# Thraix/VoxelRayTracer

Hardware: AMD Instinct MI355X
Metric: Mrays/sec + achieved HBM GB/s, 1920x1080 @ 128^3 voxels, 4 bounces (higher is better)
Workload: dtype f32

## Files before the change

voxelraytracer_amd/csrc/vrt_cert.h:

```cpp
#ifndef VRT_CERT_H
#define VRT_CERT_H

#include "vrt_walk.h"

namespace vrt {


enum : int { CERT_MISS = 0, CERT_HIT = 1, CERT_UNSURE = 2 };
constexpr int kCertRun = 3;
constexpr float kCertMargin = 1.0f / 64.0f;
constexpr int kCertMaxIter = 1024;
constexpr float kCertMaxOrigin = 4e-3f;

struct CertResult {
  int res;
  uint32_t byte;
  int axis;
  int cx, cy, cz;
  float u;
  float eu;
  float us;
  CERT_DIAG_ONLY(int iters;)
};

// ... 12 lines not shown
  uint32_t t = load_u16_at(c.vox, outside ? 0u : idx, obase);
  t = outside ? kTexOutside : t;
  asm volatile("" : "+v"(t));
  return t;
}
__device__ __forceinline__ bool cross_outside(uint32_t tex) { return tex >= kTexOutside; }
__device__ __forceinline__ uint32_t start_texel(const Ctx& c, int i, int j, int k, uint32_t obase) {
  const bool outside = max(max(uint32_t(i), uint32_t(j)), uint32_t(k)) >= uint32_t(c.n);
  const uint32_t idx = mad24(mad24(uint32_t(k), c.p, uint32_t(j)), c.p, uint32_t(i));
  const uint32_t t = load_u16_at(c.vox, outside ? 0u : idx, obase);
  return outside ? 0u : t;
}
__device__ __forceinline__ uint32_t alt_byte(const Ctx& c, int i, int j, int k, uint32_t obase) {
  const uint32_t n = uint32_t(c.n);
  if (uint32_t(i) > n || uint32_t(j) > n || uint32_t(k) > n) return 0u;
  return cell_texel(c, i, j, k, obase) & kVoxMask;
}
template <bool SHADOW>
__device__ __forceinline__ bool cert_event(uint32_t b, uint32_t medium) {
  return SHADOW ? (b & ~2u) != 0u : b != medium;
}

struct CertStartK {
  f3 Ps, fl;
  int mx, my, mz;
};
typedef const __attribute__((address_space(4))) KArgs LateKArgs;
__device__ __forceinline__ LateKArgs* late_kargs() {
  LateKArgs* ka = (LateKArgs*)__builtin_amdgcn_kernarg_segment_ptr();
  asm volatile("" : "+s"(ka));
  return ka;
}

template <bool SHADOW, bool LEAN = false, bool ED = true>
__device__ __forceinline__ CertResult cert_walk(const Ctx& c, const f3 P, const f3 D, const f3 rcp, const float U,
                                int cx, int cy, int cz, const float e0, const f3 ed,
                                const float len0b, const uint32_t medium, const uint32_t tex0 = ~0u,
                                const CertStartK* __restrict__ st0 = nullptr,
                                LateKArgs* sk = nullptr) {
  CertResult r;
  r.res = CERT_UNSURE;
  r.byte = 0u;
  r.axis = 0;
  r.cx = r.cy = r.cz = 0;
  r.u = 0.0f;
  r.eu = 0.0f;
  r.us = 0.0f;
  const bool ksun = LEAN && sk != nullptr;
  const int sx = ksun ? sk->sun_step[0] : (D.x > 0.0f ? 1 : -1), sy = ksun ? sk->sun_step[1] : (D.y > 0.0f ? 1 : -1),
            sz = ksun ? sk->sun_step[2] : (D.z > 0.0f ? 1 : -1);
  const int ux = ksun ? (sk->sun_step[0] > 0 ? 1 : 0) : (D.x > 0.0f ? 1 : 0), uy = ksun ? (sk->sun_step[1] > 0 ? 1 : 0) : (D.y > 0.0f ? 1 : 0),
            uz = ksun ? (sk->sun_step[2] > 0 ? 1 : 0) : (D.z > 0.0f ? 1 : 0);
  const f3 ar = mk(__builtin_fabsf(rcp.x), __builtin_fabsf(rcp.y), __builtin_fabsf(rcp.z));
  const float l1 = ksun ? sk->sun_l1 : __builtin_fabsf(D.x) + __builtin_fabsf(D.y) + __builtin_fabsf(D.z);
  const uint32_t obase =
      ksun ? sk->sun_obase : ((D.x < 0.0f ? 1u : 0u) | (D.y < 0.0f ? 2u : 0u) | (D.z < 0.0f ? 4u : 0u)) * c.ostride;
  constexpr float k24 = 2.0f * 0x1p-24f;
  const float q2 = ksun ? sk->sun_q2 : 0.5f * k24 * l1;
  const float lin = 6.0f + l1 * (len0b + 1.0f),
              con = (18.0f * 1.0000020f) * __builtin_amdgcn_rcpf(l1) + 3.0f * (len0b + 1.0f);
  const float a1 = k24 * (lin + 2.0f), b1 = ksun ? sk->sun_b1 : k24 * l1, b0 = k24 * (3.0f * c.fn + 11.0f);
  const float c0 = k24 * (con + 2.0f * len0b) + 4e-5f + e0;
  const float g2 = ksun ? sk->sun_g2 : 2.0f * q2, g1 = 2.0f * k24 * lin, g0 = 2.0f * k24 * con + 1e-4f + e0;
  const bool kst = LEAN && st0 != nullptr;
  const f3 Ps = kst    ? st0->Ps
                : ksun ? mk(__uint_as_float(__float_as_uint(P.x) ^ sk->sun_neg[0]), __uint_as_float(__float_as_uint(P.y) ^ sk->sun_neg[1]),
                            __uint_as_float(__float_as_uint(P.z) ^ sk->sun_neg[2]))
                       : mk(ux ? P.x : -P.x, uy ? P.y : -P.y, uz ? P.z : -P.z);
  const f3 Da = mk(__builtin_fabsf(D.x), __builtin_fabsf(D.y), __builtin_fabsf(D.z));
  const int mx = kst ? st0->mx : ux - 1, my = kst ? st0->my : uy - 1, mz = kst ? st0->mz : uz - 1;
  f3 sig = kst ? mk(((st0->fl.x + 1.0f) - Ps.x) * ar.x, ((st0->fl.y + 1.0f) - Ps.y) * ar.y,
                    ((st0->fl.z + 1.0f) - Ps.z) * ar.z)
               : mk((float(cx + ux) - P.x) * rcp.x, (float(cy + uy) - P.y) * rcp.y, (float(cz + uz) - P.z) * rcp.z);
  uint32_t tex = (tex0 != ~0u ? tex0
                              : (LEAN ? start_texel(c, cx + sx, cy + sy, cz + sz, obase)
                                      : path_texel(c, cx + sx, cy + sy, cz + sz, obase))) +
                 (1u << kDistShift);
  CTRACE(c, 100 + int(SHADOW), cx, cy, cz, P.x, P.y, P.z, U);
  CTRACE(c, 101, D.x, D.y, D.z, e0, ed.x, ed.y, ed.z);
  CERT_DIAG_ONLY(r.iters = 0;)
  if (LEAN && PHASE_STOP(SHADOW ? 4 : 2)) {
    r.u = ((sig.x + sig.y) + (sig.z + q2)) + ((a1 + b1) + (b0 + c0)) + ((g2 + g1) + (g0 + Ps.x)) +
          ((Ps.y + Ps.z) + (Da.x + Da.y)) + ((Da.z + ar.x) + (ar.y + ar.z)) + U;
    r.cx = int(tex + obase) + mx + my + mz;
    return r;
  }
  int st = CERT_UNSURE;
  for (int guard = 0; guard < kCertMaxIter; ++guard) {
    CERT_DIAG_ONLY(r.iters = guard + 1;)
    const float s1 = __builtin_fminf(sig.x, __builtin_fminf(sig.y, sig.z));
    const float uu = gmax(s1, 0.0f);
    const float A = __builtin_fmaf(__builtin_fmaf(q2, uu, a1), uu, c0);
    const float B = __builtin_fmaf(b1, uu, b0);
    auto gam_of = [&](float arb, float edb) {
      const float g = __builtin_fmaf(B, arb, A);
      return ED ? g + edb : g;
    };
    const uint32_t G = tex >> kDistShift;
    bool jumped = false;
    if (SHADOW || medium == 0u) {
      const float fg1 = float(G) - (1.0f + kCertMargin);
      const float fb = fg1 - B;
      const float jx = __builtin_fmaf(fb, ar.x, sig.x), jy = __builtin_fmaf(fb, ar.y, sig.y),
                  jz = __builtin_fmaf(fb, ar.z, sig.z);
      const float jm = ED ? __builtin_fminf(jx - ed.x, __builtin_fminf(jy - ed.y, jz - ed.z))
                          : __builtin_fminf(jx, __builtin_fminf(jy, jz));
      const float uj = __builtin_fminf(jm - A, U + 2.0f);
      CTRACE(c, 102, G, s1, uj, gam_of(ar.x, ed.x), gam_of(ar.y, ed.y), gam_of(ar.z, ed.z), 0);
      if (uj > s1) {
        const float fx = __builtin_floorf(__builtin_fmaf(uj, Da.x, Ps.x)),
                    fy = __builtin_floorf(__builtin_fmaf(uj, Da.y, Ps.y)),
                    fz = __builtin_floorf(__builtin_fmaf(uj, Da.z, Ps.z));
        cx = int(fx) ^ mx;
        cy = int(fy) ^ my;
        cz = int(fz) ^ mz;
        if constexpr (LEAN)
          sig = mk(((fx + 1.0f) - Ps.x) * ar.x, ((fy + 1.0f) - Ps.y) * ar.y, ((fz + 1.0f) - Ps.z) * ar.z);
        else
          sig = mk((float(cx + ux) - P.x) * rcp.x, (float(cy + uy) - P.y) * rcp.y, (float(cz + uz) - P.z) * rcp.z);
        tex = LEAN ? cell_texel(c, cx, cy, cz, obase) : path_texel(c, cx, cy, cz, obase);
        jumped = true;
      }
    }
    st = kCertRun;
    if (!jumped) {
      const int a = sig.x == s1 ? 0 : (sig.y == s1 ? 1 : 2);
      const f3 gam = mk(gam_of(ar.x, ed.x), gam_of(ar.y, ed.y), gam_of(ar.z, ed.z));
      const f3 back = mk(sig.x - ar.x, sig.y - ar.y, sig.z - ar.z);
      const float mback = gmax(back.x, gmax(back.y, back.z));
      const float prev = gmax(mback, 0.0f);
// ... 663 lines not shown
  const float ey = h.eu * __builtin_fabsf(dy) +
                   0x1p-21f * (__builtin_fabsf(py0) + __builtin_fabsf(h.u * dy) + __builtin_fabsf(py) + 1.0f);
  uint32_t i, j;
  if (!texel_pair(c, px, ex, mat_tex_x(m), false, i) || !texel_pair(c, py, ey, mat_tex_y(m), true, j)) return false;
  const uint32_t t = c.atlas[j * (c.atlas_mask + 1u) + i];
  col = make_float4(float(t & 0xFFu) / 255.0f, float((t >> 8) & 0xFFu) / 255.0f,
                    float((t >> 16) & 0xFFu) / 255.0f, float(t >> 24) / 255.0f);
  return true;
}

__device__ __forceinline__ void late_ctx(Ctx& c) {
  LateKArgs* ka = late_kargs();
  c.sky_sy = ka->sky_sy;
  c.sun_n = mk(ka->sun_n[0], ka->sun_n[1], ka->sun_n[2]);
  c.sun_rcp = mk(ka->sun_rcp[0], ka->sun_rcp[1], ka->sun_rcp[2]);
  c.atlas = ka->atlas;
  c.atlas_mask = uint32_t(ka->atlas_size) - 1u;
  c.atlas_fs = float(ka->atlas_size);
  c.atlas_fts = float(ka->atlas_tex_size);
}
template <bool TEX = false, bool TREE = false, int NL = kWgThreads, bool LEAN = false>
__device__ __forceinline__ bool cert_pixel(const Ctx& c0, const Ray& ray0, f3& color_out, int max_refl = 0,
                                           int max_transp = 0, float* __restrict__ ltb = nullptr,
                                           float* us_out = nullptr) {
  const f3 P = ray0.pos, D = ray0.dir;
  int cx, cy, cz;
  CertStartK st;
  if constexpr (LEAN) {
    const bool ux = D.x > 0.0f, uy = D.y > 0.0f, uz = D.z > 0.0f;
    st.Ps = mk(ux ? P.x : -P.x, uy ? P.y : -P.y, uz ? P.z : -P.z);
    st.fl = mk(__builtin_floorf(st.Ps.x), __builtin_floorf(st.Ps.y), __builtin_floorf(st.Ps.z));
    st.mx = ux ? 0 : -1;
    st.my = uy ? 0 : -1;
    st.mz = uz ? 0 : -1;
    cx = int(st.fl.x) ^ st.mx;
    cy = int(st.fl.y) ^ st.my;
    cz = int(st.fl.z) ^ st.mz;
    bool ok = int(fast_path_ok(D)) & int(max(max(uint32_t(cx), uint32_t(cy)), uint32_t(cz)) < uint32_t(c0.n)) &
              int(__builtin_floorf(st.Ps.x + 1.0f) == st.fl.x + 1.0f) &
              int(__builtin_floorf(st.Ps.y + 1.0f) == st.fl.y + 1.0f) &
              int(__builtin_floorf(st.Ps.z + 1.0f) == st.fl.z + 1.0f);
    const bool on_plane = (int(!ux) & int(st.fl.x == st.Ps.x)) | (int(!uy) & int(st.fl.y == st.Ps.y)) |
                          (int(!uz) & int(st.fl.z == st.Ps.z));
    if (ok & on_plane) ok = start_layers_clear<false>(c0, P, D, cx, cy, cz, 0u);
    if (!ok) { CERT_DIAG(0); return false; }
  } else {
    if (!fast_path_ok(D)) { CERT_DIAG(0); return false; }
    if (!exact_start_cell(c0, P, D, cx, cy, cz) || !start_layers_clear<false>(c0, P, D, cx, cy, cz, 0u)) {
      CERT_DIAG(0);
      return false;
    }
  }
  const f3 rcp = mk(__builtin_amdgcn_rcpf(D.x), __builtin_amdgcn_rcpf(D.y), __builtin_amdgcn_rcpf(D.z));
  CertResult h = cert_walk<false, LEAN, false>(c0, P, D, rcp, c0.max_len - ray0.len, cx, cy, cz, 0.0f,
                                               mk(0.0f, 0.0f, 0.0f), 0.0f, 0u, ~0u, LEAN ? &st : nullptr);
  if (us_out) *us_out = h.us;
  CERT_DIAG_ONLY(cert_diag_iters(10, h.iters);)
  if (LEAN && (PHASE_STOP(2) || PHASE_STOP(3))) {
    color_out = mk(h.u, h.eu, float(h.cx + h.cy + h.cz + h.axis + int(h.byte) + h.res));
    return true;
  }
  if (h.res == CERT_UNSURE) { CERT_DIAG(1); return false; }
  Ctx c = c0;
  if constexpr (LEAN) late_ctx(c);
  f3 color = mk(0.0f, 0.0f, 0.0f);
  if (h.res == CERT_MISS) {
    CERT_DIAG(2);
// ... 25 lines not shown
```

voxelraytracer_amd/csrc/vrt_context.cpp:

```cpp
#include <hip/hip_runtime.h>
#include <rccl/rccl.h>

#include <algorithm>
#include <cmath>
#include <cstdint>
#include <cstring>
#include <string>
#include <vector>

#include "vrt.h"
#include "vrt_internal.h"

namespace {

constexpr int kParts = 2;
constexpr int kLanes = 4;
constexpr int kOrderSlots = 16;
constexpr uint32_t kOrderMaxTiles = 1u << 17;
constexpr size_t kOrderSlotWords = vrt::kOrdHdr + 5u * size_t(kOrderMaxTiles) + 2u * vrt::kOrdClasses;
uint32_t defer_seg_tiles(uint32_t tiles, uint32_t tiles_x) {
  return (tiles_x + vrt::kOrdClasses - 1u) / vrt::kOrdClasses * (tiles / tiles_x);
}
size_t defer_words(uint32_t tiles, uint32_t tiles_x) {
  return vrt::kDeferHdr + size_t(vrt::kOrdClasses) * defer_seg_tiles(tiles, tiles_x) * vrt::kWgThreads;
}
constexpr int kRing = 8;
constexpr size_t kVstatWords = 8;
static_assert(kRing % kLanes == 0, "a ring slot is always written from the same lane");

// ... 50 lines not shown
  uint64_t order_tick = 0;
  uint32_t order_assigned = 0;
};

}

void vrt::sun_consts(KArgs& a) {
  const float* s = a.sun_n;
  const float lo = 0x1p-64f, hi = 1.0e4f;
  bool ok = true;
  for (int b = 0; b < 3; ++b) ok = ok && std::fabs(s[b]) >= lo && std::fabs(s[b]) <= hi;
  a.sun_ok = ok ? 1u : 0u;
  for (int b = 0; b < 3; ++b) {
    a.sun_neg[b] = s[b] > 0.0f ? 0u : 0x80000000u;
    a.sun_step[b] = s[b] > 0.0f ? 1 : -1;
  }
  a.sun_obase = ((s[0] < 0.0f ? 1u : 0u) | (s[1] < 0.0f ? 2u : 0u) | (s[2] < 0.0f ? 4u : 0u)) * a.ostride;
  constexpr float k24 = 2.0f * 0x1p-24f;
  const float l1 = std::fabs(s[0]) + std::fabs(s[1]) + std::fabs(s[2]);
  a.sun_l1 = l1;
  a.sun_q2 = 0.5f * k24 * l1;
  a.sun_b1 = k24 * l1;
  a.sun_g2 = 2.0f * a.sun_q2;
}

struct vrt_ctx {
  std::vector<Shard> sh;
  bool distinct = true;
  bool coll1 = false;
  std::vector<ncclComm_t> comms;
  int32_t layout_req = 0;
  int32_t cert_req = 0;
  int32_t tree_req = 1;
  int tile_order = 1;
  int32_t exact_pass = 1;
  std::vector<hipEvent_t> lt_ev;
  size_t lt_used = 0;
  std::vector<uint8_t> atlas_host;
  int32_t hist_w = 0, hist_h = 0;
  uint64_t fk = 0;
  bool raw_is_cur[kRing] = {};
  bool reset_pending = false;
  uint32_t* d_gather = nullptr;
  size_t hist_pixels_gather = 0;
  uint32_t* d_frames[kRing] = {};
  hipEvent_t ev_consumed[kRing] = {};
// ... 251 lines not shown
  a.refr_noise = p->refraction_noise;
  a.max_len = p->max_ray_length;
  a.n = s.n;
  a.fn = float(s.n);
  a.width = cam->width;
  a.height = cam->height;
  a.rcp_w = 1.0f / float(cam->width);
  a.rcp_h = 1.0f / float(cam->height);
  a.row0 = row0;
  a.rows = rows;
  a.row_step = row_step;
  a.row_blk_sh = 0;
  a.pitch = cam->width;
  a.ostride = octant_stride(s);
  vrt::sun_consts(a);
  a.max_refl = p->max_reflections;
  a.max_transp = p->max_transparencies;
  a.textured = p->color_only ? 0 : 1;
  a.atlas_size = p->color_only ? 1 : p->atlas_size;
  a.atlas_tex_size = p->atlas_texture_size;
  a.atlas = s.d_atlas;
  a.alpha = 1.0f;
  a.vdiv_ok = 0;
  a.prev = nullptr;
  a.cur = nullptr;
  a.raw = nullptr;
  const bool trees = ctx->tree_req == 2 || (ctx->tree_req == 1 && !s.cert_auto);
  a.cert = s.octants != 8 || ctx->cert_req < 0 ? 0 : (ctx->cert_req > 0 || s.cert_auto || trees ? 2 : 1);
  a.tree = a.cert == 2 && p->color_only && trees ? 1 : 0;
  a.tiles_x = uint32_t((a.width + vrt::kTileW - 1) / vrt::kTileW);
  a.tiles = a.tiles_x * uint32_t((a.rows + vrt::kTileH - 1) / vrt::kTileH);
  a.order = nullptr;
  a.ord_r = a.ord_w = a.ctr_r = a.ctr_w = a.ctr_z = a.ord_q = 0;
  a.defer = nullptr;
  a.defer_e = a.defer_seg = 0;
  a.exact_fat = 0;
  a.exact_grid = 0;
  a.batches_out = nullptr;
  a.nframes = 1;
  a.frame_tiles = a.tiles;
  std::memset(a.fb, 0, sizeof(a.fb));
  return a;
}

OrderSlot* acquire_slot(Shard& s, const vrt::KArgs& a, hipStream_t st) {
  if (a.tiles == 0 || a.tiles > kOrderMaxTiles) return nullptr;
// ... 112 lines not shown
  return slot;
}

bool vertex_div_ranges_ok(const float* m) {
  const double hi = 0x1p59, lo = 0x1p-59;
  double sum[4];
  for (int i = 0; i < 4; ++i) {
    sum[i] = std::fabs(double(m[i])) + std::fabs(double(m[4 + i])) + std::fabs(double(m[8 + i])) +
             std::fabs(double(m[12 + i]));
    if (!(sum[i] * (1.0 + 0x1p-20) <= hi)) return false;
  }
  const double side = std::fabs(double(m[3])) + std::fabs(double(m[7])) + sum[3] * 0x1p-20;
  return std::fabs(double(m[15]) - double(m[11])) - side >= lo &&
         std::fabs(double(m[15]) + double(m[11])) - side >= lo;
}

void launch(const vrt_ctx* ctx, Shard& s, vrt::KArgs a, float4* out, vrt_hit* hit, unsigned long long* cnt,
            hipStream_t st, hipEvent_t ev_begin = nullptr, hipEvent_t ev_end = nullptr, bool allow_defer = true,
            bool lone = false) {
  const bool stats = hit || cnt;
  a.vdiv_ok = vertex_div_ranges_ok(a.inv_pv) ? 1u : 0u;
  for (int f = 1; f < a.nframes; ++f)
    if (!vertex_div_ranges_ok(a.fb[f - 1].inv_pv)) a.vdiv_ok = 0u;
  OrderSlot* slot = stats ? nullptr : launch_state_begin(ctx, s, a, st, allow_defer || lone, lone);
  vrt::launch_render(a, stats, s.d_vox_pad, out, hit, cnt ? s.d_cnt_rep : nullptr, st, ev_begin, ev_end);
  slot_launched(s, slot, st);
  if (cnt) vrt::launch_reduce_counters(s.d_cnt_rep, cnt, st);
}

int volume_alloc(vrt_ctx* ctx, Shard& s, int32_t n) {
  if (n < 2 || n > 1024 || (n & (n - 1)) != 0)
    return fail(ctx, VRT_ERR_INVALID, "volume edge must be a power of two in [2, 1024]");
  VRT_HIP(ctx, hipSetDevice(s.device));
  VRT_HIP(ctx, hipDeviceSynchronize());
  const bool fits = uint64_t(n + 1) * (n + 1) * (n + 1) * 2 * 8 <= (uint64_t(1) << 32);
  const int32_t octants = fits && ctx->layout_req != 1 ? 8 : 1;
  if (s.d_vox && (s.n != n || s.octants != octants)) {
    (void)hipFree(s.d_vox);
    (void)hipFree(s.d_tmp);
    (void)hipFree(s.d_vox_pad);
    s.d_vox = s.d_tmp = nullptr;
    s.d_vox_pad = nullptr;
  }
  if (!s.d_vox) {
    const size_t bytes = size_t(n) * n * n, pbytes = size_t(n + 1) * (n + 1) * (n + 1) * 2 * size_t(octants);
    if (hipMalloc(&s.d_vox, bytes) != hipSuccess ||
// ... 439 lines not shown
  if (devs.size() > 1 && c->distinct) {
    c->comms.resize(devs.size());
    if (ncclCommInitAll(c->comms.data(), int(devs.size()), devs.data()) != ncclSuccess) {
      c->comms.clear();
      vrt_destroy(c);
      return VRT_ERR_DEVICE;
    }
  }
  *out = c;
  return VRT_OK;
}

}

extern "C" {

int vrt_debug_sun_consts(const float* sun_dir, uint32_t ostride, uint32_t* out) {
  if (!sun_dir || !out) return VRT_ERR_INVALID;
  vrt::KArgs a{};
  fill_sun(a, sun_dir);
  a.ostride = ostride;
  vrt::sun_consts(a);
  std::memcpy(out, &a.sun_ok, 12 * sizeof(uint32_t));
  return VRT_OK;
}

int vrt_create(uint32_t device_mask, vrt_ctx** out) {
  std::vector<int> devs;
  for (int d = 0; d < 32; ++d)
    if (device_mask & (1u << d)) devs.push_back(d);
  if (devs.empty()) {
    if (out) *out = nullptr;
    return VRT_ERR_INVALID;
  }
  return create(devs, out);
}

int vrt_create_devices(const int32_t* devices, int32_t count, vrt_ctx** out) {
  if (!devices || count < 1) {
    if (out) *out = nullptr;
    return VRT_ERR_INVALID;
  }
  return create(std::vector<int>(devices, devices + count), out);
}

void vrt_destroy(vrt_ctx* c) {
// ... 1199 lines not shown
```

voxelraytracer_amd/csrc/vrt_internal.h:

```cpp
#ifndef VRT_INTERNAL_H
#define VRT_INTERNAL_H

#include <hip/hip_runtime.h>

#include <cstdint>

#include "vrt.h"
#include "vrt_tuning.h"

namespace vrt {

struct KArgs {
  float inv_pv[16];
  float rcp_w, rcp_h;
  float sun[3];
  float sky_sy;
  float sun_n[3];
  float sun_rcp[3];
  float time, ray_noise, refl_noise, refr_noise, max_len;
  float fn;
  int32_t n, width, height;
  int32_t row0, rows, row_step;
  int32_t row_blk_sh;
  int32_t pitch;
// ... 8 lines not shown
  uint32_t* raw;
  int32_t cert;
  int32_t tree;
  uint32_t* order;
  uint32_t tiles_x, tiles, ord_r, ord_w, ctr_r, ctr_w, ctr_z, ord_q;
  uint32_t* defer;
  uint32_t defer_e, defer_seg;
  int32_t exact_fat;
  uint32_t exact_grid;
  uint32_t* batches_out;
  int32_t nframes;
  uint32_t frame_tiles;
  struct FrameB {
    float inv_pv[16];
    float time;
    uint32_t* cur;
    uint32_t* raw;
  } fb[7];
  uint32_t sun_ok;
  uint32_t sun_neg[3];
  int32_t sun_step[3];
  uint32_t sun_obase;
  float sun_l1, sun_q2, sun_b1, sun_g2;
};
void sun_consts(KArgs& a);
constexpr int kMaxBatch = 8;
constexpr int kWgThreads = 64 * kWgWaves;
constexpr int kTileW = kWgWaves >= 2 ? 16 : 8;
constexpr int kTileH = kWgWaves == 4 ? 16 : 8;
constexpr int kMaxStack = 17;
constexpr int kCntReplicas = 256;
constexpr uint32_t kOrdClasses = 8;
constexpr uint32_t kOrdCtrStride = 64;
constexpr uint32_t kOrdHdr = 3 * kOrdClasses * kOrdCtrStride;
__host__ __device__ inline uint32_t ord_q_for(uint32_t tiles) {
  return (tiles + kOrdClasses * kOrdDiv - 1u) / (kOrdClasses * kOrdDiv);
}
constexpr uint32_t kDeferHdr = 4 * kOrdClasses * kOrdCtrStride;
constexpr uint32_t kDeferDense = 32;


void launch_render(const KArgs& a, bool stats, const uint16_t* vox, float4* out, vrt_hit* hit,
                   unsigned long long* cnt_rep, hipStream_t s, hipEvent_t ev_begin = nullptr,
                   hipEvent_t ev_end = nullptr);
constexpr int32_t kQueryPick = 2;
void launch_ray_query(const KArgs& a, int32_t kind, const uint16_t* vox, const void* in, uint32_t count,
                      vrt_ray_hit* hits, hipStream_t s, hipEvent_t ev_begin = nullptr, hipEvent_t ev_end = nullptr);
constexpr int32_t kTraceRays = 0, kTracePixels = 1;
// ... 40 lines not shown
```

voxelraytracer_amd/csrc/vrt_math.h:

```cpp
#ifndef VRT_MATH_H
#define VRT_MATH_H

#include <hip/hip_runtime.h>

#include <cstdint>

namespace vrt {


struct f3 {
  float x, y, z;
};

__device__ __forceinline__ f3 mk(float x, float y, float z) { return f3{x, y, z}; }
__device__ __forceinline__ f3 operator+(f3 a, f3 b) { return mk(a.x + b.x, a.y + b.y, a.z + b.z); }
__device__ __forceinline__ f3 operator-(f3 a, f3 b) { return mk(a.x - b.x, a.y - b.y, a.z - b.z); }
__device__ __forceinline__ f3 operator*(f3 a, float s) { return mk(a.x * s, a.y * s, a.z * s); }
__device__ __forceinline__ f3 operator*(float s, f3 a) { return mk(s * a.x, s * a.y, s * a.z); }
__device__ __forceinline__ float dot3(f3 a, f3 b) { return a.x * b.x + a.y * b.y + a.z * b.z; }
__device__ __forceinline__ float comp(f3 a, int i) { return i == 0 ? a.x : (i == 1 ? a.y : a.z); }
__device__ __forceinline__ void set_comp(f3& a, int i, float f) {
  if (i == 0) a.x = f;
  else if (i == 1) a.y = f;
  else a.z = f;
// ... 2 lines not shown
  const uint32_t e = (__float_as_uint(d) >> 23) & 0xFFu;
  return e >= 2u && e <= 252u;
}
__device__ __forceinline__ float rcp_newton(float d) {
  const float y = __builtin_amdgcn_rcpf(d);
  return __builtin_fmaf(__builtin_fmaf(-d, y, 1.0f), y, y);
}
__device__ __forceinline__ float rcp_rn(float d) { return rcp_rn_ok(d) ? rcp_newton(d) : 1.0f / d; }
__device__ __forceinline__ bool sqrt_fix_ok(float s) {
  const uint32_t e = (__float_as_uint(s) >> 23) & 0xFFu;
  return e >= 95u && e <= 252u;
}
__device__ __forceinline__ float sqrt_fix(float s) {
  const float y = __builtin_amdgcn_sqrtf(s);
  const float ym = __uint_as_float(__float_as_uint(y) - 1u), yp = __uint_as_float(__float_as_uint(y) + 1u);
  const float rm = __builtin_fmaf(-ym, y, s), rp = __builtin_fmaf(-yp, y, s);
  const float z = rm <= 0.0f ? ym : y;
  return rp > 0.0f ? yp : z;
}
__device__ __forceinline__ float sqrt_rn(float s) { return sqrt_fix_ok(s) ? sqrt_fix(s) : __builtin_sqrtf(s); }

__device__ __forceinline__ float near_one_rsqrt(uint32_t b) {
  const uint32_t one = 0x3F800000u;
  const uint32_t r = b >= one ? (b - one < 2u ? one : one - ((b - one) & ~1u))
                              : one + (((((one - b) + 1u) >> 1) + 1u) >> 1);
  return __uint_as_float(r);
}
__device__ __forceinline__ f3 normalize3(f3 v) {
  const float s = v.x * v.x + v.y * v.y + v.z * v.z;
  const uint32_t b = __float_as_uint(s);
  const float inv = b - (0x3F800000u - 1024u) <= 2048u ? near_one_rsqrt(b) : rcp_rn(sqrt_rn(s));
  return v * inv;
}
__device__ __forceinline__ float gsign(float x) { return x > 0.0f ? 1.0f : (x < 0.0f ? -1.0f : 0.0f); }
__device__ __forceinline__ float gmin(float x, float y) { return y < x ? y : x; }
__device__ __forceinline__ float gmax(float x, float y) { return __builtin_fmaxf(x, y); }
__device__ __forceinline__ float gpow(float x, float y) { return exp2f(y * log2f(x)); }
__device__ __forceinline__ float mixf(float x, float y, float a) { return x * (1.0f - a) + y * a; }
__device__ __forceinline__ f3 reflect3(f3 i, f3 n) {
  const float s = 2.0f * dot3(n, i);
  return i - s * n;
}
__device__ __forceinline__ f3 refract3(f3 i, f3 n, float eta) {
  const float d = dot3(n, i);
  const float k = 1.0f - eta * eta * (1.0f - d * d);
  if (k < 0.0f) return mk(0.0f, 0.0f, 0.0f);
  const float s = eta * d + sqrt_rn(k);
  return eta * i - s * n;
}
__device__ __forceinline__ f3 sign3(f3 d) { return mk(gsign(d.x), gsign(d.y), gsign(d.z)); }

__device__ __forceinline__ uint32_t hash1(uint32_t x) {
  x += (x << 10u);
  x ^= (x >> 6u);
  x += (x << 3u);
  x ^= (x >> 11u);
  x += (x << 15u);
  return x;
}
__device__ __forceinline__ float random4(float x, float y, float z, float w) {
  const uint32_t h = hash1(__float_as_uint(x) ^ hash1(__float_as_uint(y)) ^
                           hash1(__float_as_uint(z)) ^ hash1(__float_as_uint(w)));
  return __uint_as_float((h & 0x007FFFFFu) | 0x3F800000u) - 1.0f;
}
__device__ __forceinline__ bool zero_noise_exact(f3 d) {
  const uint32_t nz = 0x80000000u;
  return int(__float_as_uint(d.x) != nz) & int(__float_as_uint(d.y) != nz) &
         int(__float_as_uint(d.z) != nz) & int(d.x == d.x) & int(d.y == d.y) & int(d.z == d.z);
}
__device__ __forceinline__ bool zero_noise_exact_class(f3 d) {
  constexpr int kNegZeroOrNan = 0x020 | 0x001 | 0x002;
  return !(__builtin_amdgcn_classf(d.x, kNegZeroOrNan) | __builtin_amdgcn_classf(d.y, kNegZeroOrNan) |
           __builtin_amdgcn_classf(d.z, kNegZeroOrNan));
}
template <bool LEAN = false>
__device__ __forceinline__ f3 randomize(f3 dir, f3 pos, float randomness, float seed) {
  f3 r = mk(0.0f, 0.0f, 0.0f);
  if (!(randomness == 0.0f && (LEAN ? zero_noise_exact_class(dir) : zero_noise_exact(dir)))) {
    const f3 p = mk((pos.x + dir.x) + seed, (pos.y + dir.y) + seed, (pos.z + dir.z) + seed);
    const float dx = random4(p.x, p.y, p.z, 0.0f + seed);
    const float dy = random4(p.x, p.y, p.z, 0.5f + seed);
    const float dz = random4(p.x, p.y, p.z, 1.0f + seed);
    r = mk((dx + -0.5f) * randomness, (dy + -0.5f) * randomness, (dz + -0.5f) * randomness);
  }
  return normalize3(dir + r);
}


__device__ __forceinline__ uint32_t mat_id(uint32_t b) { return b > 3 ? 3 : b; }
__device__ __forceinline__ float mat_refr(uint32_t b) { return mat_id(b) == 2 ? 1.5f : 1.0f; }
__device__ __forceinline__ bool mat_transparent(uint32_t m) { return m == 0 || m == 2; }
__device__ __forceinline__ bool mat_reflective(uint32_t m) { return m == 2; }
__device__ __forceinline__ float mat_kd(uint32_t m) { return m == 0 ? 0.0f : (m == 2 ? 1.0f : 0.4f); }
__device__ __forceinline__ float mat_ks(uint32_t m, bool tex) {
  return m == 0 ? 0.0f : (m == 2 ? 1.0f : (tex ? (m == 1 ? 0.6f : 0.4f) : 0.2f));
}
__device__ __forceinline__ float mat_exp(uint32_t m, bool tex) {
  return m == 0 ? 0.0f : (m == 2 ? (tex ? 0.3f : 1.0f) : (tex ? (m == 1 ? 60.0f : 20.0f) : 10.0f));
}
__device__ __forceinline__ uint32_t mat_tex_x(uint32_t m) { return m == 3 ? 1u : 0u; }
__device__ __forceinline__ uint32_t mat_tex_y(uint32_t m) { return m >= 2 ? 1u : 0u; }
__device__ __forceinline__ float4 mat_color(uint32_t m) {
  if (m == 1) return make_float4(0.5f, 0.5f, 0.5f, 1.0f);
  if (m == 3) return make_float4(0.05f, 0.5f, 0.1f, 1.0f);
  return make_float4(0.0f, 0.0f, 0.0f, 0.0f);
}

constexpr float kAmbient = 0.3f;
// ... 7 lines not shown
```

voxelraytracer_amd/csrc/vrt_render.hip:

```cpp
#include <hip/hip_ext.h>
#include <hip/hip_runtime.h>

#include <algorithm>
#include <cmath>
#include <cstdint>
#include <cstdio>
#include <cstring>
#include <string>
#include <vector>

#include "vrt.h"
#include "vrt_internal.h"
#include "vrt_diag.h"
#include "vrt_math.h"
#include "vrt_walk.h"
#include "vrt_cert.h"
#include "vrt_aux_kernels.h"
#include "vrt_skipfield_kernels.h"

namespace vrt {

__device__ __forceinline__ uint32_t unorm8(float f) {
  const float c = __builtin_fminf(__builtin_fmaxf(f, 0.0f), 1.0f);
  return uint32_t(__builtin_rintf(c * 255.0f));
// ... 95 lines not shown
  c.refr_noise = a.refr_noise;
  if constexpr (LATE) {
    c.sky_sy = 0.0f;
    c.sun_n = c.sun_rcp = mk(0.0f, 0.0f, 0.0f);
    c.atlas = nullptr;
    c.atlas_mask = 0u;
    c.atlas_fs = c.atlas_fts = 0.0f;
  } else {
    c.sky_sy = a.sky_sy;
    c.sun_n = mk(a.sun_n[0], a.sun_n[1], a.sun_n[2]);
    c.sun_rcp = mk(a.sun_rcp[0], a.sun_rcp[1], a.sun_rcp[2]);
    c.atlas = a.atlas;
    c.atlas_mask = uint32_t(a.atlas_size) - 1u;
    c.atlas_fs = float(a.atlas_size);
    c.atlas_fts = float(a.atlas_tex_size);
  }
  CTRACE_ONLY(c.tr = false;)
}

__device__ __forceinline__ bool markstein_safe(float x) {
  const float m = __builtin_fabsf(x);
  return m >= 0x1p-60f && m <= 0x1p60f;
}
template <bool LEAN = false>
__device__ __forceinline__ f3 div3_rn(float x, float y, float z, float d, bool ranges_ok = false) {
  bool safe;
  if constexpr (LEAN) {
    bool rest = true;
    if (!ranges_ok)
      rest = int(__builtin_fabsf(x) <= 0x1p60f) & int(__builtin_fabsf(y) <= 0x1p60f) &
             int(__builtin_fabsf(z) <= 0x1p60f) & int(markstein_safe(d));
    safe = rest & (__builtin_fminf(__builtin_fminf(__builtin_fabsf(x), __builtin_fabsf(y)), __builtin_fabsf(z)) >=
                   0x1p-60f);
  } else {
    safe = markstein_safe(x) && markstein_safe(y) && markstein_safe(z) && markstein_safe(d);
  }
  if (safe) {
    const float r = rcp_newton(d);
    return mk(div_rn(x, d, r), div_rn(y, d, r), div_rn(z, d, r));
  }
  return mk(x / d, y / d, z / d);
}

template <bool LEAN = false>
__device__ __forceinline__ Ray primary_ray(const KArgs& a, const float* __restrict__ inv_pv, const Ctx& c, int px,
                                           int py) {
  const float ndx = div_rn(2.0f * (float(px) + 0.5f), float(a.width), a.rcp_w) - 1.0f;
  const float ndy = div_rn(2.0f * (float(py) + 0.5f), float(a.height), a.rcp_h) - 1.0f;
  float n4[4], f4[4];
#pragma unroll
  for (int i = 0; i < 4; ++i) {
    const float base = inv_pv[0 * 4 + i] * ndx + inv_pv[1 * 4 + i] * ndy;
    n4[i] = (base + inv_pv[2 * 4 + i] * -1.0f) + inv_pv[3 * 4 + i] * 1.0f;
    f4[i] = (base + inv_pv[2 * 4 + i] * 1.0f) + inv_pv[3 * 4 + i] * 1.0f;
  }
  const bool ranges_ok = LEAN && a.vdiv_ok != 0u;
  const f3 vnear = div3_rn<LEAN>(n4[0], n4[1], n4[2], n4[3], ranges_ok);
  const f3 vdir = div3_rn<LEAN>(f4[0], f4[1], f4[2], f4[3], ranges_ok) - vnear;
  Ray ray;
  ray.pos = mk(vnear.x + c.fn * 0.5f, vnear.y + c.fn * 0.5f, vnear.z + c.fn * 0.5f);
  ray.dir = randomize<LEAN>(normalize3(vdir), vnear, a.ray_noise, c.time);
  ray.len = 0.0f;
  ray.energy = 1.0f;
  ray.voxel = 0;
  ray.rdepth = 0;
  ray.tdepth = 0;
  return ray;
}

constexpr int kStackPrio = 3;

struct StackRay {
  f3 pos, dir;
  float len, energy;
  uint32_t depths;
};
__device__ __forceinline__ StackRay pack_stack_ray(const Ray& r) {
  return StackRay{r.pos, r.dir, r.len, r.energy, uint32_t(r.rdepth) | (uint32_t(r.tdepth) << 16)};
}
constexpr int kStackWords = 9;
template <int NL>
__device__ __forceinline__ void lds_stack_put(float* __restrict__ b, const StackRay& e) {
  b[0 * NL] = e.pos.x;
  b[1 * NL] = e.pos.y;
// ... 146 lines not shown
    constexpr int kPool = std::max(kAxFloats + kStkFloats, 4);
    __shared__ float4 lds_pool[kPool / 4];
    c.ax = &lds_pool[threadIdx.x * kAxLane];
    const Ray ray = primary_ray<DEFER>(a, FB ? frame_view(a, fr).pv : a.inv_pv, c, px, frame_row(a, li));
    k.c[VRT_CNT_PIXELS] = 1;
    k.c[VRT_CNT_PRIMARY_RAYS] = 1;
    uint32_t steps = 0, flags = 0;
    int32_t hit_vidx = -1;
    float hit_len = 0.0f;
    f3 color;
    if constexpr (!DEFER) color = mk(0.0f, 0.0f, 0.0f);
    float* tstk = nullptr;
    if constexpr (TREE) {
      static_assert(CERT == 2 && !TEX && !STATS, "certified trees: stats-free colour-only certified instances");
      tstk = reinterpret_cast<float*>(lds_pool) + kAxFloats + threadIdx.x;
    }
    float us = -1.0f;
    bool need_exact;
    if (DEFER && (PHASE_STOP(0) || PHASE_STOP(1))) {
      color = PHASE_STOP(1) ? mk(ray.pos.x + ray.dir.x, ray.pos.y + ray.dir.y, ray.pos.z + ray.dir.z)
                            : mk(0.0f, 0.0f, 0.0f);
      need_exact = false;
    } else {
      need_exact = CERT < 2 || !cert_pixel<TEX, TREE, kWgThreads, DEFER>(c, ray, color, a.max_refl, a.max_transp, tstk, &us);
    }
    STAMP_WAVE_CERT(need_exact);
    if constexpr (DEFER) {
      deferred = need_exact;
    } else if (need_exact) {
      color = mk(0.0f, 0.0f, 0.0f);
      heavy = true;
      float* lstk = reinterpret_cast<float*>(lds_pool) + kAxFloats;
      (void)exact_pixel<STATS, TEX, CERT >= 1, CERT == 2>(a, c, ray, color, k, steps, flags, hit_vidx,
                                                         hit_len, &lstk[threadIdx.x], STATS ? -1.0f : us);
    }
    const uint32_t l2 = lane_id();
    const size_t o = size_t(pixel_row(ty, wave, l2)) * size_t(a.pitch) + size_t(pixel_x(tx, wave, l2));
    if (STATS && hits) {
      vrt_hit hr;
      hr.voxel_index = hit_vidx;
      hr.ray_length = hit_len;
      hr.steps = steps;
      hr.flags = flags;
      hits[o] = hr;
    }
    if constexpr (DEFER) {
      if (!deferred) {
// ... 416 lines not shown
```

Baseline: 100,800.

## Precompute camera-invariant ray setup constants on host and pass via kernel args

After: 106,200 (median of 6 runs). +5.3%, better.

```diff
diff --git a/voxelraytracer_amd/csrc/vrt_cert.h b/voxelraytracer_amd/csrc/vrt_cert.h
--- a/voxelraytracer_amd/csrc/vrt_cert.h
+++ b/voxelraytracer_amd/csrc/vrt_cert.h
@@ -58,8 +58,9 @@
 }
 
 struct CertStartK {
-  f3 Ps, fl;
+  f3 Ps, fl1;
   int mx, my, mz;
+  float b0, U2;
 };
 typedef const __attribute__((address_space(4))) KArgs LateKArgs;
 __device__ __forceinline__ LateKArgs* late_kargs() {
@@ -83,6 +84,7 @@
   r.eu = 0.0f;
   r.us = 0.0f;
   const bool ksun = LEAN && sk != nullptr;
+  const bool kst = LEAN && st0 != nullptr;
   const int sx = ksun ? sk->sun_step[0] : (D.x > 0.0f ? 1 : -1), sy = ksun ? sk->sun_step[1] : (D.y > 0.0f ? 1 : -1),
             sz = ksun ? sk->sun_step[2] : (D.z > 0.0f ? 1 : -1);
   const int ux = ksun ? (sk->sun_step[0] > 0 ? 1 : 0) : (D.x > 0.0f ? 1 : 0), uy = ksun ? (sk->sun_step[1] > 0 ? 1 : 0) : (D.y > 0.0f ? 1 : 0),
@@ -95,18 +97,17 @@
   const float q2 = ksun ? sk->sun_q2 : 0.5f * k24 * l1;
   const float lin = 6.0f + l1 * (len0b + 1.0f),
               con = (18.0f * 1.0000020f) * __builtin_amdgcn_rcpf(l1) + 3.0f * (len0b + 1.0f);
-  const float a1 = k24 * (lin + 2.0f), b1 = ksun ? sk->sun_b1 : k24 * l1, b0 = k24 * (3.0f * c.fn + 11.0f);
+  const float a1 = k24 * (lin + 2.0f), b1 = ksun ? sk->sun_b1 : k24 * l1,
+              b0 = kst ? st0->b0 : (ksun ? sk->walk_b0 : k24 * (3.0f * c.fn + 11.0f));
   const float c0 = k24 * (con + 2.0f * len0b) + 4e-5f + e0;
   const float g2 = ksun ? sk->sun_g2 : 2.0f * q2, g1 = 2.0f * k24 * lin, g0 = 2.0f * k24 * con + 1e-4f + e0;
-  const bool kst = LEAN && st0 != nullptr;
   const f3 Ps = kst    ? st0->Ps
                 : ksun ? mk(__uint_as_float(__float_as_uint(P.x) ^ sk->sun_neg[0]), __uint_as_float(__float_as_uint(P.y) ^ sk->sun_neg[1]),
                             __uint_as_float(__float_as_uint(P.z) ^ sk->sun_neg[2]))
                        : mk(ux ? P.x : -P.x, uy ? P.y : -P.y, uz ? P.z : -P.z);
   const f3 Da = mk(__builtin_fabsf(D.x), __builtin_fabsf(D.y), __builtin_fabsf(D.z));
   const int mx = kst ? st0->mx : ux - 1, my = kst ? st0->my : uy - 1, mz = kst ? st0->mz : uz - 1;
-  f3 sig = kst ? mk(((st0->fl.x + 1.0f) - Ps.x) * ar.x, ((st0->fl.y + 1.0f) - Ps.y) * ar.y,
-                    ((st0->fl.z + 1.0f) - Ps.z) * ar.z)
+  f3 sig = kst ? mk((st0->fl1.x - Ps.x) * ar.x, (st0->fl1.y - Ps.y) * ar.y, (st0->fl1.z - Ps.z) * ar.z)
                : mk((float(cx + ux) - P.x) * rcp.x, (float(cy + uy) - P.y) * rcp.y, (float(cz + uz) - P.z) * rcp.z);
   uint32_t tex = (tex0 != ~0u ? tex0
                               : (LEAN ? start_texel(c, cx + sx, cy + sy, cz + sz, obase)
@@ -141,7 +142,7 @@
                   jz = __builtin_fmaf(fb, ar.z, sig.z);
       const float jm = ED ? __builtin_fminf(jx - ed.x, __builtin_fminf(jy - ed.y, jz - ed.z))
                           : __builtin_fminf(jx, __builtin_fminf(jy, jz));
-      const float uj = __builtin_fminf(jm - A, U + 2.0f);
+      const float uj = __builtin_fminf(jm - A, kst ? st0->U2 : U + 2.0f);
       CTRACE(c, 102, G, s1, uj, gam_of(ar.x, ed.x), gam_of(ar.y, ed.y), gam_of(ar.z, ed.z), 0);
       if (uj > s1) {
         const float fx = __builtin_floorf(__builtin_fmaf(uj, Da.x, Ps.x)),
@@ -851,27 +852,39 @@
 template <bool TEX = false, bool TREE = false, int NL = kWgThreads, bool LEAN = false>
 __device__ __forceinline__ bool cert_pixel(const Ctx& c0, const Ray& ray0, f3& color_out, int max_refl = 0,
                                            int max_transp = 0, float* __restrict__ ltb = nullptr,
-                                           float* us_out = nullptr) {
+                                           float* us_out = nullptr, const KArgs* ak = nullptr) {
   const f3 P = ray0.pos, D = ray0.dir;
   int cx, cy, cz;
   CertStartK st;
   if constexpr (LEAN) {
     const bool ux = D.x > 0.0f, uy = D.y > 0.0f, uz = D.z > 0.0f;
     st.Ps = mk(ux ? P.x : -P.x, uy ? P.y : -P.y, uz ? P.z : -P.z);
-    st.fl = mk(__builtin_floorf(st.Ps.x), __builtin_floorf(st.Ps.y), __builtin_floorf(st.Ps.z));
     st.mx = ux ? 0 : -1;
     st.my = uy ? 0 : -1;
     st.mz = uz ? 0 : -1;
-    cx = int(st.fl.x) ^ st.mx;
-    cy = int(st.fl.y) ^ st.my;
-    cz = int(st.fl.z) ^ st.mz;
-    bool ok = int(fast_path_ok(D)) & int(max(max(uint32_t(cx), uint32_t(cy)), uint32_t(cz)) < uint32_t(c0.n)) &
-              int(__builtin_floorf(st.Ps.x + 1.0f) == st.fl.x + 1.0f) &
-              int(__builtin_floorf(st.Ps.y + 1.0f) == st.fl.y + 1.0f) &
-              int(__builtin_floorf(st.Ps.z + 1.0f) == st.fl.z + 1.0f);
-    const bool on_plane = (int(!ux) & int(st.fl.x == st.Ps.x)) | (int(!uy) & int(st.fl.y == st.Ps.y)) |
-                          (int(!uz) & int(st.fl.z == st.Ps.z));
-    if (ok & on_plane) ok = start_layers_clear<false>(c0, P, D, cx, cy, cz, 0u);
+    st.b0 = ak->walk_b0;
+    st.U2 = ak->max_len2;
+    bool ok;
+    if ((ak->setup & kSetupCell) != 0u) {
+      st.fl1 = mk(ux ? ak->start_fl1[0] : ak->start_fl1[3], uy ? ak->start_fl1[1] : ak->start_fl1[4],
+                  uz ? ak->start_fl1[2] : ak->start_fl1[5]);
+      cx = ak->start_cell[0];
+      cy = ak->start_cell[1];
+      cz = ak->start_cell[2];
+      ok = fast_path_ok(D);
+    } else {
+      const f3 fl = mk(__builtin_floorf(st.Ps.x), __builtin_floorf(st.Ps.y), __builtin_floorf(st.Ps.z));
+      st.fl1 = mk(fl.x + 1.0f, fl.y + 1.0f, fl.z + 1.0f);
+      cx = int(fl.x) ^ st.mx;
+      cy = int(fl.y) ^ st.my;
+      cz = int(fl.z) ^ st.mz;
+      ok = int(fast_path_ok(D)) & int(max(max(uint32_t(cx), uint32_t(cy)), uint32_t(cz)) < uint32_t(c0.n)) &
+           int(__builtin_floorf(st.Ps.x + 1.0f) == st.fl1.x) & int(__builtin_floorf(st.Ps.y + 1.0f) == st.fl1.y) &
+           int(__builtin_floorf(st.Ps.z + 1.0f) == st.fl1.z);
+      const bool on_plane = (int(!ux) & int(fl.x == st.Ps.x)) | (int(!uy) & int(fl.y == st.Ps.y)) |
+                            (int(!uz) & int(fl.z == st.Ps.z));
+      if (ok & on_plane) ok = start_layers_clear<false>(c0, P, D, cx, cy, cz, 0u);
+    }
     if (!ok) { CERT_DIAG(0); return false; }
   } else {
     if (!fast_path_ok(D)) { CERT_DIAG(0); return false; }
diff --git a/voxelraytracer_amd/csrc/vrt_context.cpp b/voxelraytracer_amd/csrc/vrt_context.cpp
--- a/voxelraytracer_amd/csrc/vrt_context.cpp
+++ b/voxelraytracer_amd/csrc/vrt_context.cpp
@@ -5,6 +5,7 @@
 #include <cmath>
 #include <cstdint>
 #include <cstring>
+#include <limits>
 #include <string>
 #include <vector>
 
@@ -101,6 +102,82 @@
   a.sun_q2 = 0.5f * k24 * l1;
   a.sun_b1 = k24 * l1;
   a.sun_g2 = 2.0f * a.sun_q2;
+}
+
+void vrt::setup_consts(KArgs& a) {
+  constexpr float k24 = 2.0f * 0x1p-24f;
+  a.fw = float(a.width);
+  a.fh = float(a.height);
+  a.half_n = a.fn * 0.5f;
+  a.walk_b0 = k24 * (3.0f * a.fn + 11.0f);
+  a.max_len2 = a.max_len + 2.0f;
+}
+
+void vrt::cert_launch_consts(KArgs& a) {
+  a.setup = 0u;
+  a.wn = a.wf = a.rcp_wn = a.rcp_wf = 0.0f;
+  for (int i = 0; i < 6; ++i) a.start_fl1[i] = 0.0f;
+  for (int b = 0; b < 3; ++b) a.start_cell[b] = 0;
+  if (a.vdiv_ok == 0u) return;
+  for (int f = 1; f < a.nframes; ++f)
+    if (std::memcmp(a.fb[f - 1].inv_pv, a.inv_pv, sizeof(a.inv_pv)) != 0) return;
+  const float* m = a.inv_pv;
+  for (int i = 0; i < 16; ++i)
+    if (!std::isfinite(m[i])) return;
+
+  const double am11 = std::fabs(double(m[11]));
+  if (!(am11 >= double(std::numeric_limits<float>::min()))) return;
+  const double ulp = std::ldexp(1.0, std::ilogb(am11) - 23);
+  if (!((std::fabs(double(m[3])) + std::fabs(double(m[7]))) * (1.0 + 0x1p-20) < ulp * 0.25)) return;
+  const float wn = -m[11] + m[15], wf = m[11] + m[15];
+  const auto markstein = [](float x) { return std::fabs(x) >= 0x1p-60f && std::fabs(x) <= 0x1p60f; };
+  if (!markstein(wn) || !markstein(wf)) return;
+  a.wn = wn;
+  a.wf = wf;
+  a.rcp_wn = 1.0f / wn;
+  a.rcp_wf = 1.0f / wf;
+  a.setup |= kSetupW;
+
+  const double iwn = 1.0 / std::fabs(double(wn)), iwf = 1.0 / std::fabs(double(wf));
+  double S[3], en[3], ev1 = 0.0, up = 0.0;
+  double ca[3], cb[3], cc[3];
+  for (int b = 0; b < 3; ++b) {
+    S[b] = std::fabs(double(m[b])) + std::fabs(double(m[4 + b])) + std::fabs(double(m[8 + b])) +
+           std::fabs(double(m[12 + b]));
+    en[b] = 0x1p-19 * S[b] * iwn;
+    const double ef = 0x1p-19 * S[b] * iwf;
+    ev1 += 2.0 * (en[b] + ef);
+    up += S[b] * (iwn + iwf);
+    const double d = 1.0 / double(wf) - 1.0 / double(wn);
+    ca[b] = double(m[b]) * d;
+    cb[b] = double(m[4 + b]) * d;
+    cc[b] = (double(m[8 + b]) + double(m[12 + b])) / double(wf) - (double(m[12 + b]) - double(m[8 + b])) / double(wn);
+  }
+
+  const double cl = std::sqrt(cc[0] * cc[0] + cc[1] * cc[1] + cc[2] * cc[2]);
+  if (cl > 0.0 && std::isfinite(cl)) {
+    const double pa = std::fabs(ca[0] * cc[0] + ca[1] * cc[1] + ca[2] * cc[2]) / cl;
+    const double pb = std::fabs(cb[0] * cc[0] + cb[1] * cc[1] + cb[2] * cc[2]) / cl;
+    if (cl - pa - pb - ev1 >= 4.0 && up + ev1 <= 0x1p49) a.setup |= kSetupLen;
+  }
+
+  const double half = double(a.fn) * 0.5;
+  int32_t cell[3];
+  for (int b = 0; b < 3; ++b) {
+    const double centre = (double(m[12 + b]) - double(m[8 + b])) / double(wn) + half;
+    const double spread = (std::fabs(double(m[b])) + std::fabs(double(m[4 + b]))) * iwn;
+    const double e = en[b] + 0x1p-23 * (std::fabs(centre) + half + spread) + 0x1p-9;
+    const double lo = centre - spread - e, hi = centre + spread + e;
+    const double c = std::floor(lo);
+    if (!(lo > c && hi < c + 1.0 && c >= 0.0 && c < double(a.n))) return;
+    cell[b] = int32_t(c);
+  }
+  for (int b = 0; b < 3; ++b) {
+    a.start_cell[b] = cell[b];
+    a.start_fl1[b] = float(cell[b] + 1);
+    a.start_fl1[3 + b] = float(-cell[b]);
+  }
+  a.setup |= kSetupCell;
 }
 
 struct vrt_ctx {
@@ -398,6 +475,8 @@
   a.atlas = s.d_atlas;
   a.alpha = 1.0f;
   a.vdiv_ok = 0;
+  vrt::setup_consts(a);
+  vrt::cert_launch_consts(a);
   a.prev = nullptr;
   a.cur = nullptr;
   a.raw = nullptr;
@@ -556,6 +635,13 @@
   a.vdiv_ok = vertex_div_ranges_ok(a.inv_pv) ? 1u : 0u;
   for (int f = 1; f < a.nframes; ++f)
     if (!vertex_div_ranges_ok(a.fb[f - 1].inv_pv)) a.vdiv_ok = 0u;
+  vrt::cert_launch_consts(a);
+#ifdef VRT_SETUP_MASK
+#ifndef VRT_DIAGNOSTIC_BUILD
+#error "VRT_SETUP_MASK is a diagnostic build: use make variant"
+#endif
+  a.setup &= uint32_t(VRT_SETUP_MASK);
+#endif
   OrderSlot* slot = stats ? nullptr : launch_state_begin(ctx, s, a, st, allow_defer || lone, lone);
   vrt::launch_render(a, stats, s.d_vox_pad, out, hit, cnt ? s.d_cnt_rep : nullptr, st, ev_begin, ev_end);
   slot_launched(s, slot, st);
@@ -1041,6 +1127,34 @@
   a.ostride = ostride;
   vrt::sun_consts(a);
   std::memcpy(out, &a.sun_ok, 12 * sizeof(uint32_t));
+  return VRT_OK;
+}
+
+int vrt_debug_cert_launch_consts(const float* inv_pv, const float* inv_pv2, int32_t n, int32_t width, int32_t height,
+                                 float max_len, uint32_t* out) {
+  if (!inv_pv || !out) return VRT_ERR_INVALID;
+  vrt::KArgs a{};
+  std::memcpy(a.inv_pv, inv_pv, sizeof(a.inv_pv));
+  a.n = n;
+  a.fn = float(n);
+  a.width = width;
+  a.height = height;
+  a.max_len = max_len;
+  a.nframes = 1;
+  a.vdiv_ok = vertex_div_ranges_ok(a.inv_pv) ? 1u : 0u;
+  if (inv_pv2) {
+    a.nframes = 2;
+    std::memcpy(a.fb[0].inv_pv, inv_pv2, sizeof(a.inv_pv));
+    if (!vertex_div_ranges_ok(a.fb[0].inv_pv)) a.vdiv_ok = 0u;
+  }
+  vrt::setup_consts(a);
+  vrt::cert_launch_consts(a);
+  out[0] = a.setup;
+  std::memcpy(out + 1, &a.wn, 4 * sizeof(float));
+  std::memcpy(out + 5, a.start_fl1, 6 * sizeof(float));
+  std::memcpy(out + 11, a.start_cell, 3 * sizeof(int32_t));
+  std::memcpy(out + 14, &a.fw, 5 * sizeof(float));
+  out[19] = a.vdiv_ok;
   return VRT_OK;
 }
 
diff --git a/voxelraytracer_amd/csrc/vrt_internal.h b/voxelraytracer_amd/csrc/vrt_internal.h
--- a/voxelraytracer_amd/csrc/vrt_internal.h
+++ b/voxelraytracer_amd/csrc/vrt_internal.h
@@ -54,8 +54,16 @@
   int32_t sun_step[3];
   uint32_t sun_obase;
   float sun_l1, sun_q2, sun_b1, sun_g2;
+  float fw, fh, half_n, walk_b0, max_len2;
+  uint32_t setup;
+  float wn, wf, rcp_wn, rcp_wf;
+  float start_fl1[6];
+  int32_t start_cell[3];
 };
+constexpr uint32_t kSetupW = 1u, kSetupLen = 2u, kSetupCell = 4u;
 void sun_consts(KArgs& a);
+void setup_consts(KArgs& a);
+void cert_launch_consts(KArgs& a);
 constexpr int kMaxBatch = 8;
 constexpr int kWgThreads = 64 * kWgWaves;
 constexpr int kTileW = kWgWaves >= 2 ? 16 : 8;
diff --git a/voxelraytracer_amd/csrc/vrt_math.h b/voxelraytracer_amd/csrc/vrt_math.h
--- a/voxelraytracer_amd/csrc/vrt_math.h
+++ b/voxelraytracer_amd/csrc/vrt_math.h
@@ -48,15 +48,16 @@
 
 __device__ __forceinline__ float near_one_rsqrt(uint32_t b) {
   const uint32_t one = 0x3F800000u;
-  const uint32_t r = b >= one ? (b - one < 2u ? one : one - ((b - one) & ~1u))
-                              : one + (((((one - b) + 1u) >> 1) + 1u) >> 1);
+  const uint32_t r = b >= one ? one - ((b - one) & ~1u) : one + (((((one - b) + 1u) >> 1) + 1u) >> 1);
   return __uint_as_float(r);
+}
+__device__ __forceinline__ float normalize3_scale(float s) {
+  const uint32_t b = __float_as_uint(s);
+  return b - (0x3F800000u - 1024u) <= 2048u ? near_one_rsqrt(b) : rcp_rn(sqrt_rn(s));
 }
 __device__ __forceinline__ f3 normalize3(f3 v) {
   const float s = v.x * v.x + v.y * v.y + v.z * v.z;
-  const uint32_t b = __float_as_uint(s);
-  const float inv = b - (0x3F800000u - 1024u) <= 2048u ? near_one_rsqrt(b) : rcp_rn(sqrt_rn(s));
-  return v * inv;
+  return v * normalize3_scale(s);
 }
 __device__ __forceinline__ float gsign(float x) { return x > 0.0f ? 1.0f : (x < 0.0f ? -1.0f : 0.0f); }
 __device__ __forceinline__ float gmin(float x, float y) { return y < x ? y : x; }
@@ -102,14 +103,16 @@
 template <bool LEAN = false>
 __device__ __forceinline__ f3 randomize(f3 dir, f3 pos, float randomness, float seed) {
   f3 r = mk(0.0f, 0.0f, 0.0f);
+  f3 sum = dir;
   if (!(randomness == 0.0f && (LEAN ? zero_noise_exact_class(dir) : zero_noise_exact(dir)))) {
     const f3 p = mk((pos.x + dir.x) + seed, (pos.y + dir.y) + seed, (pos.z + dir.z) + seed);
     const float dx = random4(p.x, p.y, p.z, 0.0f + seed);
     const float dy = random4(p.x, p.y, p.z, 0.5f + seed);
     const float dz = random4(p.x, p.y, p.z, 1.0f + seed);
     r = mk((dx + -0.5f) * randomness, (dy + -0.5f) * randomness, (dz + -0.5f) * randomness);
+    sum = dir + r;
   }
-  return normalize3(dir + r);
+  return normalize3(LEAN ? sum : dir + r);
 }
 
 
diff --git a/voxelraytracer_amd/csrc/vrt_render.hip b/voxelraytracer_amd/csrc/vrt_render.hip
--- a/voxelraytracer_amd/csrc/vrt_render.hip
+++ b/voxelraytracer_amd/csrc/vrt_render.hip
@@ -141,44 +141,78 @@
   const float m = __builtin_fabsf(x);
   return m >= 0x1p-60f && m <= 0x1p60f;
 }
-template <bool LEAN = false>
-__device__ __forceinline__ f3 div3_rn(float x, float y, float z, float d, bool ranges_ok = false) {
-  bool safe;
-  if constexpr (LEAN) {
-    bool rest = true;
-    if (!ranges_ok)
-      rest = int(__builtin_fabsf(x) <= 0x1p60f) & int(__builtin_fabsf(y) <= 0x1p60f) &
-             int(__builtin_fabsf(z) <= 0x1p60f) & int(markstein_safe(d));
-    safe = rest & (__builtin_fminf(__builtin_fminf(__builtin_fabsf(x), __builtin_fabsf(y)), __builtin_fabsf(z)) >=
-                   0x1p-60f);
-  } else {
-    safe = markstein_safe(x) && markstein_safe(y) && markstein_safe(z) && markstein_safe(d);
-  }
-  if (safe) {
+__device__ __forceinline__ f3 div3_rn(float x, float y, float z, float d) {
+  if (markstein_safe(x) && markstein_safe(y) && markstein_safe(z) && markstein_safe(d)) {
     const float r = rcp_newton(d);
     return mk(div_rn(x, d, r), div_rn(y, d, r), div_rn(z, d, r));
   }
   return mk(x / d, y / d, z / d);
+}
+__device__ __forceinline__ f3 div3_lean(float x, float y, float z, float d, float r, bool rest) {
+  const bool safe = rest & (__builtin_fminf(__builtin_fminf(__builtin_fabsf(x), __builtin_fabsf(y)), __builtin_fabsf(z)) >=
+                            0x1p-60f);
+  if (safe) return mk(div_rn(x, d, r), div_rn(y, d, r), div_rn(z, d, r));
+  return mk(x / d, y / d, z / d);
+}
+__device__ __forceinline__ bool div3_lean_ranges(float x, float y, float z, float d) {
+  return int(__builtin_fabsf(x) <= 0x1p60f) & int(__builtin_fabsf(y) <= 0x1p60f) & int(__builtin_fabsf(z) <= 0x1p60f) &
+         int(markstein_safe(d));
 }
 
 template <bool LEAN = false>
 __device__ __forceinline__ Ray primary_ray(const KArgs& a, const float* __restrict__ inv_pv, const Ctx& c, int px,
                                            int py) {
-  const float ndx = div_rn(2.0f * (float(px) + 0.5f), float(a.width), a.rcp_w) - 1.0f;
-  const float ndy = div_rn(2.0f * (float(py) + 0.5f), float(a.height), a.rcp_h) - 1.0f;
+  const float ndx = div_rn(2.0f * (float(px) + 0.5f), LEAN ? a.fw : float(a.width), a.rcp_w) - 1.0f;
+  const float ndy = div_rn(2.0f * (float(py) + 0.5f), LEAN ? a.fh : float(a.height), a.rcp_h) - 1.0f;
   float n4[4], f4[4];
 #pragma unroll
-  for (int i = 0; i < 4; ++i) {
+  for (int i = 0; i < (LEAN ? 3 : 4); ++i) {
     const float base = inv_pv[0 * 4 + i] * ndx + inv_pv[1 * 4 + i] * ndy;
     n4[i] = (base + inv_pv[2 * 4 + i] * -1.0f) + inv_pv[3 * 4 + i] * 1.0f;
     f4[i] = (base + inv_pv[2 * 4 + i] * 1.0f) + inv_pv[3 * 4 + i] * 1.0f;
   }
-  const bool ranges_ok = LEAN && a.vdiv_ok != 0u;
-  const f3 vnear = div3_rn<LEAN>(n4[0], n4[1], n4[2], n4[3], ranges_ok);
-  const f3 vdir = div3_rn<LEAN>(f4[0], f4[1], f4[2], f4[3], ranges_ok) - vnear;
+  f3 vnear, vdir;
+  if constexpr (LEAN) {
+    float rn, rf;
+    bool rest_n = true, rest_f = true;
+    if ((a.setup & kSetupW) != 0u) {
+      n4[3] = a.wn;
+      f4[3] = a.wf;
+      rn = a.rcp_wn;
+      rf = a.rcp_wf;
+    } else {
+      const float base = inv_pv[0 * 4 + 3] * ndx + inv_pv[1 * 4 + 3] * ndy;
+      n4[3] = (base + inv_pv[2 * 4 + 3] * -1.0f) + inv_pv[3 * 4 + 3] * 1.0f;
+      f4[3] = (base + inv_pv[2 * 4 + 3] * 1.0f) + inv_pv[3 * 4 + 3] * 1.0f;
+      if (a.vdiv_ok == 0u) {
+        rest_n = div3_lean_ranges(n4[0], n4[1], n4[2], n4[3]);
+        rest_f = div3_lean_ranges(f4[0], f4[1], f4[2], f4[3]);
+      }
+      rn = rcp_newton(n4[3]);
+      rf = rcp_newton(f4[3]);
+    }
+    vnear = div3_lean(n4[0], n4[1], n4[2], n4[3], rn, rest_n);
+    vdir = div3_lean(f4[0], f4[1], f4[2], f4[3], rf, rest_f) - vnear;
+  } else {
+    vnear = div3_rn(n4[0], n4[1], n4[2], n4[3]);
+    vdir = div3_rn(f4[0], f4[1], f4[2], f4[3]) - vnear;
+  }
   Ray ray;
-  ray.pos = mk(vnear.x + c.fn * 0.5f, vnear.y + c.fn * 0.5f, vnear.z + c.fn * 0.5f);
-  ray.dir = randomize<LEAN>(normalize3(vdir), vnear, a.ray_noise, c.time);
+  const float half_n = LEAN ? a.half_n : c.fn * 0.5f;
+  ray.pos = mk(vnear.x + half_n, vnear.y + half_n, vnear.z + half_n);
+  f3 dir0;
+  if constexpr (LEAN) {
+    const float s = vdir.x * vdir.x + vdir.y * vdir.y + vdir.z * vdir.z;
+    float inv;
+    if ((a.setup & kSetupLen) != 0u)
+      inv = rcp_newton(sqrt_fix(s));
+    else
+      inv = normalize3_scale(s);
+    dir0 = vdir * inv;
+  } else {
+    dir0 = normalize3(vdir);
+  }
+  ray.dir = randomize<LEAN>(dir0, vnear, a.ray_noise, c.time);
   ray.len = 0.0f;
   ray.energy = 1.0f;
   ray.voxel = 0;
@@ -371,7 +405,7 @@
                             : mk(0.0f, 0.0f, 0.0f);
       need_exact = false;
     } else {
-      need_exact = CERT < 2 || !cert_pixel<TEX, TREE, kWgThreads, DEFER>(c, ray, color, a.max_refl, a.max_transp, tstk, &us);
+      need_exact = CERT < 2 || !cert_pixel<TEX, TREE, kWgThreads, DEFER>(c, ray, color, a.max_refl, a.max_transp, tstk, &us, &a);
     }
     STAMP_WAVE_CERT(need_exact);
     if constexpr (DEFER) {
```
